# Luckick/EAGCN

Hardware: AMD Instinct MI355X
Metric: molecules/sec fwd+bwd, 2-layer 5-view EAGCN, Tox21 batch (higher is better)
Workload: dtype f32 (bf16x3 split, fp32 accumulate): every fp32 operand leaves its producer as three bf16 planes, six v_mfma_f32_32x32x16_bf16 piece products per 16 k rebuild the fp32 product (csrc/gemm_bx3.hip); aggregation, BatchNorm, head, first layer fp32

## Files before the change

eagcn_amd/_lib.py:

```python
import ctypes as C
import os

_HERE = os.path.dirname(os.path.abspath(__file__))
LIB_PATH = os.path.join(_HERE, 'lib', 'libeagcn_hip.so')

MAX_VIEWS = 8
MAX_SEGS = 8
META_WORDS = 16
META_NLOG = 8
META_T, META_NMAX, META_NTILES, META_BAD_ADJ, META_BAD_REL, META_NEDGE, META_OVERFLOW, META_EDGE_OVERFLOW = range(8)
META_NBLK = 9
STRUCT_CONCATE, STRUCT_WEIGHTED = 0, 1

_fp = C.c_void_p


class Batch(C.Structure):
    _fields_ = [('B', C.c_int32), ('N', C.c_int32), ('K', C.c_int32), ('ldc', C.c_int32),
                ('T', C.c_int32), ('n_max', C.c_int32), ('n_tiles', C.c_int32),
                ('channels', C.c_int32 * MAX_VIEWS),
                ('code', _fp), ('deg_bn', _fp), ('nat', _fp), ('row0', _fp), ('tile0', _fp),
                ('meta', _fp), ('row_mol', _fp), ('row_loc', _fp), ('row_m', _fp), ('row_deg', _fp),
                ('tile_mol', _fp), ('row_info', _fp), ('tile_info', _fp),
                ('rel_vec', _fp * MAX_VIEWS), ('rel_c', C.c_int32 * MAX_VIEWS),
# ... 72 lines not shown

class HeadGrads(C.Structure):
    _fields_ = [(n, _fp) for n in ('d_den1_w', 'd_den2_w', 'd_den3_w', 'd_gbn_w', 'd_gbn_b', 'd_bn1_w', 'd_bn1_b',
                                   'd_bn2_w', 'd_bn2_b')]


class Model(C.Structure):
    _fields_ = [('n_layers', C.c_int32), ('molfp_mode', C.c_int32), ('training', C.c_int32),
                ('head_seed', C.c_uint64), ('head_seed_dev', _fp), ('input_packed', C.c_int32), ('aux_stream', _fp),
                ('layer', LayerParams * 4), ('head', HeadParams), ('stats_hook', _fp), ('stats_user', _fp),
                ('stats_world', C.c_int32), ('fuse_readout', C.c_int32), ('fwd_signal', _fp), ('wait_flag', _fp), ('start_signal', _fp)]


class StepLoss(C.Structure):
    _fields_ = [('kind', C.c_int32), ('labels', _fp), ('class_weight', _fp), ('loss', _fp), ('scale', _fp), ('dout', _fp)]


ALLREDUCE_FN = C.CFUNCTYPE(C.c_int, C.c_void_p, C.c_int, C.c_void_p, C.c_void_p)


SIGNATURES = {
    'eagcn_abi_version': (C.c_int, []),
    'eagcn_struct_size': (C.c_size_t, [C.c_int]),
    'eagcn_last_error': (C.c_char_p, []),
    'eagcn_pad16': (C.c_int, [C.c_int]),
    'eagcn_layer_out_ld': (C.c_int, [C.POINTER(LayerParams)]),
    'eagcn_layer_fp': (C.c_int, [C.POINTER(LayerParams)]),
    'eagcn_layer_packed_bytes': (C.c_size_t, [C.POINTER(Batch), C.POINTER(LayerParams)]),
    'eagcn_layer_fwd_scratch_bytes': (C.c_size_t, [C.POINTER(Batch), C.POINTER(LayerParams)]),
    'eagcn_layer_bwd_scratch_bytes': (C.c_size_t, [C.POINTER(Batch), C.POINTER(LayerParams)]),
    'eagcn_index_build': (C.c_int, [_fp, C.POINTER(_fp), C.POINTER(Batch), _fp, _fp]),
    'eagcn_index_from_bonds': (C.c_int, [_fp, _fp, _fp, _fp, C.c_int64, C.POINTER(Batch), _fp, _fp]),
    'eagcn_index_rows': (C.c_int, [C.POINTER(Batch), _fp]),
    'eagcn_set_gemm_mode': (C.c_int, [C.c_int]),
    'eagcn_stream_wait_counter': (C.c_int, [_fp, C.c_uint32, _fp]),
    'eagcn_stream_signal_flag': (C.c_int, [_fp, _fp]),
    'eagcn_stream_wait_flag': (C.c_int, [_fp, C.c_double, _fp]),
    'eagcn_stream_wait_timeouts': (C.c_int, []),
    'eagcn_stream_wait_reset': (None, []),
    'eagcn_adam_step': (C.c_int, [_fp, _fp, _fp, _fp, C.c_int64, _fp, _fp, _fp, _fp]),
    'eagcn_agg_wants_bond_lists': (C.c_int, [C.c_int, C.c_int]),
    'eagcn_agg_wants_bond_lists_for': (C.c_int, [C.c_int, C.c_int, C.c_int]),
    'eagcn_bx3_used_splits': (C.c_int, [C.c_int, C.c_int, C.c_int, C.c_int]),
    'eagcn_set_bx3_wide': (C.c_int, [C.c_int]),
    'eagcn_bx3_pair_used_splits': (C.c_int, [C.c_int] * 7),
    'eagcn_bx3_plane_elems': (C.c_size_t, [C.c_int, C.c_int]),
    'eagcn_bx3_split': (C.c_int, [_fp, C.c_int, C.c_int, _fp, C.c_size_t, C.c_int, C.c_int, _fp]),
    'eagcn_gemm_bx3': (C.c_int, [C.c_int, C.c_int, C.c_int, C.c_int, _fp, C.c_size_t, C.c_int, C.c_int, _fp, C.c_size_t, C.c_int, C.c_int,
# ... 99 lines not shown
        return _lib
    if not os.path.exists(LIB_PATH):
        raise EagcnHipError(
            'libeagcn_hip.so is not built (%s). Run `python -c "import __graft_entry__ as g; g.build()"` '
            'or `python -m eagcn_amd.build`; eagcn_amd has no CPU fallback.' % LIB_PATH)
    lib = C.CDLL(LIB_PATH)
    lib.eagcn_abi_version.restype = C.c_int
    if lib.eagcn_abi_version() != ABI_VERSION:
        raise EagcnHipError('libeagcn_hip.so speaks ABI version %d, this binding version %d: rebuild it '
                            '(`python -c "import __graft_entry__ as g; g.build()"`)' % (lib.eagcn_abi_version(), ABI_VERSION))
    for name, (res, args) in SIGNATURES.items():
        fn = getattr(lib, name)
        fn.restype = res
        fn.argtypes = args
    for which, cls in ((0, Batch), (1, Layout), (2, LayerParams), (3, LayerBufs), (4, LayerGrads), (5, HeadParams), (6, HeadGrads),
                       (7, Model), (10, StepLoss)):
        if lib.eagcn_struct_size(which) != C.sizeof(cls):
            raise EagcnHipError('ABI mismatch: %s is %d bytes here, %d in libeagcn_hip.so'
                                % (cls.__name__, C.sizeof(cls), lib.eagcn_struct_size(which)))
    _lib = lib
    return lib


def check(rc, what):
    if rc != 0:
        msg = load().eagcn_last_error()
        raise EagcnHipError('%s failed (%d): %s' % (what, rc, msg.decode() if msg else '?'))


def pad16(w):
    return (int(w) + 15) & ~15
# ... 14 lines not shown
```

eagcn_amd/csrc/api.cpp:

```cpp
#include <hip/hip_runtime_api.h>
#include <stdarg.h>
#include <stdint.h>
#include <stdio.h>

#include <vector>

#include "../../include/eagcn_hip.h"

namespace eagcn {
static thread_local char g_err[1024] = "";
void set_error(const char* fmt, ...) {
    va_list ap;
    va_start(ap, fmt);
    vsnprintf(g_err, sizeof(g_err), fmt, ap);
    va_end(ap);
}

hipEvent_t pool_event() {
    static std::vector<hipEvent_t> pool;
    static size_t next = 0;
    constexpr size_t kPool = 256;
    if (pool.empty()) {
        pool.resize(kPool, nullptr);
        for (auto& e : pool)
// ... 59 lines not shown

extern "C" int eagcn_abi_version(void) { return 7; }
extern "C" size_t eagcn_struct_size(int which) {
    switch (which) {
        case 0: return sizeof(eagcn_batch);
        case 1: return sizeof(eagcn_layout);
        case 2: return sizeof(eagcn_layer_params);
        case 3: return sizeof(eagcn_layer_bufs);
        case 4: return sizeof(eagcn_layer_grads);
        case 5: return sizeof(eagcn_head_params);
        case 6: return sizeof(eagcn_head_grads);
        case 7: return sizeof(eagcn_model);
        case 8: return sizeof(eagcn_gat_params);
        case 9: return sizeof(eagcn_pool_att);
        case 10: return sizeof(eagcn_step_loss);
        default: return 0;
    }
}
extern "C" const char* eagcn_last_error(void) { return eagcn::g_err; }
```

eagcn_amd/csrc/head.hip:

```cpp
#include <stdlib.h>

#include <algorithm>

#include "common.h"
#include "kernels.h"

namespace eagcn {

__global__ void wait_counter_kernel(const uint32_t* __restrict__ word, uint32_t value, int* __restrict__ err,
                                    unsigned long long budget_ticks) {
    if (threadIdx.x == 0) {
        const unsigned long long t0 = wall_clock64();
        while ((int32_t)(__hip_atomic_load(word, __ATOMIC_ACQUIRE, __HIP_MEMORY_SCOPE_AGENT) - value) < 0) {
            __builtin_amdgcn_s_sleep(64);
            if (wall_clock64() - t0 > budget_ticks) {
                if (err) __hip_atomic_store(err, 1, __ATOMIC_RELAXED, __HIP_MEMORY_SCOPE_SYSTEM);
                break;
            }
        }
    }
}



// ... 225 lines not shown
    EAGCN_CHECK_ARG(carve_saved(saved, b, m, &sv) <= saved_bytes, "eagcn_model_atom_rep_materialize: saved block too small");
    const int l = m->n_layers - 1;
    LayerSaved& L = sv.L[l];
    eagcn_layer_bufs w;
    memset(&w, 0, sizeof(w));
    w.Y = L.Y; w.bn = L.bn; w.xout = L.xout; w.pad_row = L.pad_row; w.packed = L.packed; w.packed_bytes = L.packed_bytes;
    return layer_apply_impl(b, &m->layer[l], &w, stream);
}

extern "C" int eagcn_model_pack_input(const eagcn_batch* b, const eagcn_model* m, const float* afm, void* saved,
                                      size_t saved_bytes, void* stream) {
    EAGCN_CHECK_ARG(b && m && afm && saved, "eagcn_model_pack_input: null argument");
    ModelSaved sv;
    EAGCN_CHECK_ARG(carve_saved(saved, b, m, &sv) <= saved_bytes, "eagcn_model_pack_input: saved block too small");
    return eagcn_pack_rows(b, afm, layout_width(&m->layer[0].in), &m->layer[0].in, sv.x0, stream);
}

struct HeadPlan {
    HeadFwd f1, f2, f3;
    HeadBwd b3, b2, b1;
    HeadGbn bg;
    double *st_g, *st_1, *st_2, *sb_g, *sb_1, *sb_2;
    bool sync;
};
static HeadPlan head_plan(const eagcn_batch* b, const eagcn_model* m, const ModelSaved& sv, const ModelScratch& sc, float* out,
                          float* graph_rep, const float* dout, const float* dgraph_rep, const eagcn_head_grads* hg) {
    HeadPlan P;
    const eagcn_head_params* h = &m->head;
    const int B = b->B, F = h->f_in, n1 = h->n_den1, n2 = h->n_den2, nc = h->nclass;
    P.st_g = sc.hst; P.st_1 = sc.hst + 2 * F + 2; P.st_2 = sc.hst + 2 * (F + n1) + 4;
// ... 500 lines not shown
```

eagcn_amd/csrc/index.hip:

```cpp
#include <algorithm>

#include <stdlib.h>

#include "common.h"
#include "kernels.h"

namespace eagcn {

struct RelPtrs {
    const float* p[EAGCN_MAX_VIEWS];
    int c[EAGCN_MAX_VIEWS];
};

template <int NIT, int RPW>
__global__ __launch_bounds__(256) void index_scan_kernel(const float* __restrict__ adj, RelPtrs rel,
                                                          int B, int N, int Ncap, int K, int ldc,
                                                          uint8_t* __restrict__ code,
                                                          int32_t* __restrict__ deg_bn,
                                                          int32_t* __restrict__ nat,
                                                          int32_t* __restrict__ ecnt,
                                                          int32_t* __restrict__ meta) {
    const int lane = threadIdx.x & 63;
    const long row_first = ((long)blockIdx.x * 4 + (threadIdx.x >> 6)) * RPW;
    const long nrows = (long)B * N;
// ... 414 lines not shown
        bt.row_loc[r0 + i] = i;
        bt.row_deg[r0 + i] = d;
        bt.row_m[r0 + i] = d > 0 ? 1.0f : 0.0f;
        reinterpret_cast<int4*>(bt.row_info)[r0 + i] = make_int4(b, i, n, r0);
    }
    for (int t = threadIdx.x; t < (n + 15) / 16 && t0 + t < bt.n_tiles; t += blockDim.x) {
        bt.tile_mol[t0 + t] = b;
        reinterpret_cast<int4*>(bt.tile_info)[t0 + t] = make_int4(b, t, n, r0);
    }
    if (threadIdx.x == 0 && bt.mol_info) {
        const int e0 = bt.edge0[b];
        reinterpret_cast<int4*>(bt.mol_info)[b] = make_int4(r0 + n <= bt.T ? n : 0, r0, e0, bt.edge0[b + 1] - e0);
    }
}

__device__ __forceinline__ void index_blocks_body(const eagcn_batch& bt, const int rb, const int lane) {
    const int T = bt.meta[EAGCN_META_T];
    int4* out = reinterpret_cast<int4*>(bt.blk);
    int nb = 0, start = 0, rows = 0, cnt = 0;
    int start_r0 = 0, start_e0 = 0;
    auto close = [&](int end, int end_e0) {
        if (lane == 0) {
            out[2 * nb] = make_int4(start, end - start, start_r0, rows);
            out[2 * nb + 1] = make_int4(start_e0, end_e0 - start_e0, 0, 0);
        }
        ++nb; rows = 0; cnt = 0;
    };
    int last_e0 = 0;
    for (int base = 0; base < bt.B && T > 0; base += 64) {
        const int nv = min(64, bt.B - base);
// ... 182 lines not shown
    return -1;
}

__global__ __launch_bounds__(256) void pack_rows_kernel(eagcn_batch bt, const float* __restrict__ dense,
                                                         int F, ColMap m, int ld, float* __restrict__ packed, int Nin) {
    const uint32_t total = (uint32_t)dev_rows(bt) * (uint32_t)ld;
    for (uint32_t e = blockIdx.x * blockDim.x + threadIdx.x; e < total; e += gridDim.x * blockDim.x) {
        int r = (int)(e / (uint32_t)ld), cp = (int)(e - (uint32_t)r * (uint32_t)ld);
        int ce = packed_to_exact(m, cp);
        float v = 0.0f;
        if (ce >= 0) v = dense[((size_t)bt.row_mol[r] * Nin + bt.row_loc[r]) * F + ce];
        packed[e] = v;
    }
}

__global__ __launch_bounds__(256) void pad_rows_kernel(const float* __restrict__ rows, const int32_t* __restrict__ off,
                                                        int B, int N, int F, float* __restrict__ out) {
    const size_t total = (size_t)B * N * F;
    for (size_t e = (size_t)blockIdx.x * blockDim.x + threadIdx.x; e < total; e += (size_t)gridDim.x * blockDim.x) {
        const int f = (int)(e % F);
        const size_t bi = e / F;
        const int i = (int)(bi % N), b = (int)(bi / N);
        const int o = off[b], n = off[b + 1] - o;
        out[e] = i < n ? rows[(size_t)(o + i) * F + f] : 0.0f;
    }
}

__global__ __launch_bounds__(256) void unpack_rows_kernel(eagcn_batch bt, const float* __restrict__ packed,
                                                           ColMap m, int ld, const float* __restrict__ pad_row,
                                                           float* __restrict__ dense, int F) {
// ... 8 lines not shown
            if (ce < eo + m.w[s]) { cp = po + (ce - eo); break; }
            eo += m.w[s];
            po += m.p[s];
        }
        float v;
        if (i < bt.nat[b]) v = packed[(size_t)(bt.row0[b] + i) * ld + cp];
        else v = pad_row ? pad_row[cp] : 0.0f;
        dense[e] = v;
    }
}

}

using namespace eagcn;

extern "C" int eagcn_index_build(const float* adj, const float* const* rel, eagcn_batch* b,
                                 int32_t* host_meta, void* stream) {
    hipStream_t s = (hipStream_t)stream;
    EAGCN_CHECK_ARG(adj && rel && b && host_meta, "eagcn_index_build: null argument");
    EAGCN_CHECK_ARG(b->B > 0 && b->N > 0, "eagcn_index_build: B and N must be positive");
    EAGCN_CHECK_ARG(b->K >= 1 && b->K <= EAGCN_MAX_VIEWS, "eagcn_index_build: K=%d out of range", b->K);
    EAGCN_CHECK_ARG(b->ldc >= b->N && (b->ldc % 16) == 0, "eagcn_index_build: ldc must be a multiple of 16 >= N");
    EAGCN_CHECK_ARG(b->code && b->deg_bn && b->nat && b->row0 && b->tile0 && b->meta,
                    "eagcn_index_build: index buffers not allocated");
    RelPtrs rp;
    for (int k = 0; k < EAGCN_MAX_VIEWS; ++k) {
        rp.p[k] = k < b->K ? rel[k] : nullptr;
        rp.c[k] = k < b->K ? b->channels[k] : 0;
        if (k < b->K) {
            EAGCN_CHECK_ARG(rel[k] != nullptr, "eagcn_index_build: relation tensor %d is null", k);
            EAGCN_CHECK_ARG(rp.c[k] >= 1 && rp.c[k] <= EAGCN_MAX_CHANNELS,
                            "eagcn_index_build: view %d has %d channels (1..%d supported)", k, rp.c[k],
// ... 26 lines not shown
#undef EAGCN_SCAN4
#undef EAGCN_SCAN4_AL
        EAGCN_LAUNCH_CHECK();
    } else
    {
#define EAGCN_SCAN(NIT) index_scan_kernel<NIT, RPW><<<sgrid, 256, 0, s>>>(adj, rp, b->B, Nin, b->N, b->K, b->ldc, b->code, b->deg_bn, b->nat, b->ecnt, b->meta)
        switch (nit) {
            case 1: EAGCN_SCAN(1); break;
            case 2: EAGCN_SCAN(2); break;
            case 3: EAGCN_SCAN(3); break;
            default: EAGCN_SCAN(4); break;
        }
#undef EAGCN_SCAN
        EAGCN_LAUNCH_CHECK();
    }
    index_offsets_kernel<<<1, 1024, 0, s>>>(b->nat, b->B, b->deg_bn, b->B * b->N, b->row0, b->tile0, b->meta, b->T, b->ecnt, b->edge0, b->E, b->n_logical > 0 ? b->n_logical : 0);
    EAGCN_LAUNCH_CHECK();
    EAGCN_HIP(hipMemcpyAsync(host_meta, b->meta, EAGCN_META_WORDS * sizeof(int32_t), hipMemcpyDeviceToHost, s));
    return EAGCN_OK;
}

extern "C" int eagcn_index_from_bonds(const int32_t* bond_mol, const int32_t* bond_i, const int32_t* bond_j,
                                      const uint8_t* bond_code, int64_t E, eagcn_batch* b, int32_t* host_meta,
                                      void* stream) {
    hipStream_t s = (hipStream_t)stream;
    EAGCN_CHECK_ARG(b && host_meta, "eagcn_index_from_bonds: null argument");
    EAGCN_CHECK_ARG(E == 0 || (bond_mol && bond_i && bond_j && bond_code), "eagcn_index_from_bonds: null bond arrays");
    EAGCN_CHECK_ARG(b->B > 0 && b->N > 0 && b->K >= 1 && b->K <= EAGCN_MAX_VIEWS, "eagcn_index_from_bonds: bad batch shape");
    EAGCN_CHECK_ARG(b->ldc >= b->N && (b->ldc % 16) == 0, "eagcn_index_from_bonds: ldc must be a multiple of 16 >= N");
    EAGCN_CHECK_ARG(b->code && b->deg_bn && b->nat && b->row0 && b->tile0 && b->meta,
                    "eagcn_index_from_bonds: index buffers not allocated");
    RelPtrs rp;
    for (int k = 0; k < EAGCN_MAX_VIEWS; ++k) { rp.p[k] = nullptr; rp.c[k] = k < b->K ? b->channels[k] : 0; }
    ProfScope ps(PROF_INDEX, s);
    EAGCN_CHECK_ARG(b->ecnt && b->edge0, "eagcn_index_from_bonds: bond-list buffers not allocated");
    EAGCN_CHECK_ARG((long)b->B * b->N < (1L << 31), "eagcn_index_from_bonds: B * N = %ld rows", (long)b->B * b->N);
    {
        const int rcz = index_clear(b->meta, b->nat, b->ecnt, b->B, b->deg_bn, (long)b->B * b->N, s);
        if (rcz) return rcz;
    }
    EAGCN_HIP(hipMemsetAsync(b->code, 0, (size_t)b->K * b->B * b->N * b->ldc, s));
    if (E > 0) {
        const int grid = (int)std::min<long>((E + 255) / 256, 4096);
        index_bonds_kernel<<<grid, 256, 0, s>>>(bond_mol, bond_i, bond_j, bond_code, (long)E, b->B, b->N,
                                                b->n_logical > 0 ? std::min(b->n_logical, b->N) : b->N, b->K, b->ldc, rp,
                                                b->code, b->deg_bn, b->nat, b->ecnt, b->meta);
        EAGCN_LAUNCH_CHECK();
    }
    index_offsets_kernel<<<1, 1024, 0, s>>>(b->nat, b->B, b->deg_bn, b->B * b->N, b->row0, b->tile0, b->meta, b->T, b->ecnt, b->edge0, b->E, b->n_logical > 0 ? b->n_logical : 0);
    EAGCN_LAUNCH_CHECK();
    EAGCN_HIP(hipMemcpyAsync(host_meta, b->meta, EAGCN_META_WORDS * sizeof(int32_t), hipMemcpyDeviceToHost, s));
    return EAGCN_OK;
}

extern "C" int eagcn_index_rows(const eagcn_batch* b, void* stream) {
    hipStream_t s = (hipStream_t)stream;
    EAGCN_CHECK_ARG(b, "eagcn_index_rows: null batch");
    if (b->T == 0) return EAGCN_OK;
    EAGCN_CHECK_ARG(b->row_mol && b->row_loc && b->row_m && b->row_deg && b->tile_mol && b->row_info && b->tile_info,
                    "eagcn_index_rows: per-row buffers not allocated");
    EAGCN_CHECK_ARG(b->N <= 1024, "eagcn_index_rows: N=%d exceeds the supported 1024 atoms", b->N);
    EAGCN_CHECK_ARG(b->edge0 && b->mol_info && b->row_ptr && b->col_ptr && (b->E == 0 || (b->nbr && b->tnbr && b->ecode && b->tcode)),
                    "eagcn_index_rows: bond-list buffers not allocated");
    ProfScope ps(PROF_INDEX, s);
    index_rows_kernel<<<b->B, 256, 0, s>>>(*b);
    EAGCN_LAUNCH_CHECK();
    if (!b->build_lists) return EAGCN_OK;
    const int rb = b->blk ? lagg_block_rows(b) : 0;
    const int W = (b->N + 31) / 32;
    const size_t dyn = (size_t)2 * b->N * W * sizeof(uint32_t);
    static const size_t lds_cap = [] {
        int dev = 0, v = 0;
        if (hipGetDevice(&dev) != hipSuccess || hipDeviceGetAttribute(&v, hipDeviceAttributeMaxSharedMemoryPerBlock, dev) != hipSuccess) v = 64 * 1024;
        size_t cap = (size_t)v > 12 * 1024 ? (size_t)v - 12 * 1024 : 0;
        if (cap > 52 * 1024 &&
            hipFuncSetAttribute((const void*)index_csr_kernel<true>, hipFuncAttributeMaxDynamicSharedMemorySize, (int)cap) != hipSuccess) {
            (void)hipGetLastError();
            cap = 52 * 1024;
        }
        return cap;
    }();
    if (b->N <= 512 && dyn <= lds_cap) index_csr_kernel<true><<<b->B + (rb > 0 ? 1 : 0), 256, dyn, s>>>(*b, W, rb);
    else index_csr_kernel<false><<<b->B + (rb > 0 ? 1 : 0), 256, 0, s>>>(*b, W, rb);
    EAGCN_LAUNCH_CHECK();
    return EAGCN_OK;
}

extern "C" int eagcn_pack_rows(const eagcn_batch* b, const float* dense, int F, const eagcn_layout* lay,
                               float* packed, void* stream) {
    hipStream_t s = (hipStream_t)stream;
    EAGCN_CHECK_ARG(b && dense && lay && packed, "eagcn_pack_rows: null argument");
    EAGCN_CHECK_ARG(layout_width(lay) == F, "eagcn_pack_rows: layout width %d != F %d", layout_width(lay), F);
    if (b->T == 0) return EAGCN_OK;
    int ld = layout_ld(lay);
    size_t total = (size_t)b->T * ld;
    int grid = (int)std::min<size_t>((total + 255) / 256, 4096);
    ProfScope ps(PROF_PACK, s);
    pack_rows_kernel<<<grid, 256, 0, s>>>(*b, dense, F, make_colmap(lay), ld, packed, b->n_logical > 0 ? b->n_logical : b->N);
    EAGCN_LAUNCH_CHECK();
    return EAGCN_OK;
}
// ... 26 lines not shown
```

eagcn_amd/csrc/kernels.h:

```cpp
#pragma once
#include "bx3.h"
#include "common.h"

namespace eagcn {

struct AggArgs {
    eagcn_batch bt;
    ViewCols vc;
    const float* src; int lds;
    float* dst; int ldd;
    const float* sig;
    const float* rsig;
    float* rscale;
    double* stats;
    int nchunk;
    int cpw = 1;
    int xcd = 0;
    bool w_rowm = false;
    BxOut planes = {nullptr, 0, 0, 0};
    const float* bn_tab = nullptr; const float* bn_cc = nullptr; int bn_fp = 0;
    const float* w_aw = nullptr;
    int w_drop = 0; uint32_t w_thr = 0; float w_inv_keep = 1.0f; uint64_t w_seed = 0; const uint64_t* w_seed_dev = nullptr;
};
int agg_grid_x(const eagcn_batch* b);
bool agg_ksplit(const eagcn_batch* b);
int launch_agg(AggArgs a, bool trans, hipStream_t s);
constexpr int LAGG_RB = 256;
constexpr int LAGG_MAXM = 16;
struct EdgeArgs;
int lagg_parts();
bool lagg_wfuse();
bool lagg_use(const eagcn_batch* b, int dir, bool absorbs_bn, const ViewCols* vc = nullptr);
bool lagg_wanted(int B, int N, int structure);
int lagg_block_rows(const eagcn_batch* b);
int lagg_slabs(const eagcn_batch* b);
int launch_lagg_fwd(AggArgs a, hipStream_t s);
int launch_lagg_bwd(AggArgs a, const EdgeArgs& e, hipStream_t s, bool edge = true);
int launch_lagg_bwd_input(const AggArgs& a, const EdgeArgs& e, dim3 grid, hipStream_t s);

struct EdgeArgs {
    eagcn_batch bt;
    ViewCols vc;
    const float* dY; const float* Y; const float* P; int ld;
    const float* sig; const float* rsig; const float* rscale;
    double* datt;
    int atomic;
    int xcd = 0;
};
constexpr int EDGE_SLAB = 264;
constexpr int EDGE_COPIES = 8;
inline size_t edge_acc_bytes() { return align256((size_t)EDGE_COPIES * EAGCN_MAX_VIEWS * EDGE_SLAB * sizeof(double)); }
// ... 192 lines not shown
```

eagcn_amd/graph.py:

```python
import ctypes as C
import os

import torch

from . import _lib as L
from . import ops
from .ops import _index_stream, _ptr, _stream

_RING = 4
_SIDE_AFTER_FWD = os.environ.get('EAGCN_SIDE_AFTER_FWD', '1') == '1'
_SIDE_PLACED = os.environ.get('EAGCN_SIDE_PLACED', '0')
_SIDE_PLACED_MAX_ROWS = int(os.environ.get('EAGCN_SIDE_PLACED_MAX_ROWS', '40000'))
_REQUIRE_IN_GRAPH = os.environ.get('EAGCN_REQUIRE_IN_GRAPH_ALLREDUCE', '0') == '1'
_COMM_IN_GRAPH = os.environ.get('EAGCN_COMM_IN_GRAPH', '1') != '0'
_CAPTURE_DRAIN_S = float(os.environ.get('EAGCN_CAPTURE_DRAIN_S', '0.35'))


_READY_FLAG = os.environ.get('EAGCN_READY_FLAG', '1') != '0'
_flag_tested = {}


def _ready_flag_ok(device):
    if not _READY_FLAG:
        return False
    key = device.index if device.index is not None else torch.cuda.current_device()
    if key not in _flag_tested:
        lib = L.load()
        flag = torch.zeros(1, dtype=torch.int32, device=device)
        torch.cuda.synchronize(device)
        main, side = torch.cuda.current_stream(device), _index_stream(device)
        L.check(lib.eagcn_stream_wait_flag(C.c_void_p(flag.data_ptr()), 0.05, C.c_void_p(main.cuda_stream)), 'eagcn_stream_wait_flag')
        L.check(lib.eagcn_stream_signal_flag(C.c_void_p(flag.data_ptr()), C.c_void_p(side.cuda_stream)), 'eagcn_stream_signal_flag')
        torch.cuda.synchronize(device)
# ... 91 lines not shown
        self.generation = 0
        self.size_static = [torch.ones(B, dtype=torch.int64, device=device) for _ in range(2)]
        self.aux = None
        self.dp_group = None
        if os.environ.get('EAGCN_AUX_STREAM', '0') == '1':
            self.aux = torch.cuda.Stream(device=self.device)
        self.fwd_sig = torch.zeros(1, dtype=torch.int32, device=device)
        self.side_placed = _SIDE_PLACED == '1' or (_SIDE_PLACED == 'auto' and B * N <= _SIDE_PLACED_MAX_ROWS)
        self.ready = torch.zeros(2, dtype=torch.int32, device=device)
        self.use_flag = _ready_flag_ok(device)
        self.start_word = torch.zeros(1, dtype=torch.int32, device=device)
        self.starts_issued = 0
        self.markers = [None, None]
        self.fwd_issued = 0
        self.cms = [self._cmodel(i) for i in range(2)]
        m = self.cms[0]
        self.saved_bytes = lib.eagcn_model_saved_bytes(self.index.ref(), C.byref(m))
        self.scratch_bytes = lib.eagcn_model_scratch_bytes(self.index.ref(), C.byref(m))
        self.saved = [torch.empty(self.saved_bytes, dtype=torch.uint8, device=device) for _ in range(2)]
        self.scratch = torch.empty(self.scratch_bytes, dtype=torch.uint8, device=device)
        if plan.stats is not None:
            from .parallel import register_stats_buffer
            register_stats_buffer(self.scratch)
        f32 = dict(dtype=torch.float32, device=device)
        self.out = torch.zeros((B, m.head.nclass), **f32)
        self.graph_rep = torch.zeros((B, m.head.n_den2), **f32)
        self.dout = torch.zeros((B, m.head.nclass), **f32)
        self.dgr = torch.zeros((B, m.head.n_den2), **f32)
        self.dgr_is_zero = True
        self._weight_src = None
# ... 158 lines not shown
        lib = L.load()
        self._check_old_batches()
        self.cur = cur = self.step % 2
        idx = self.index = self.slots[cur]
        main = torch.cuda.current_stream(self.device)
        slot = self.step % _RING
        if self.meta_event[slot] is not None:
            self._check_old_batches(force=True, only=slot)
        if self.use_flag:
            slot_free = ('count', self.starts_issued) if self.starts_issued >= 2 else None
        else:
            ev = torch.cuda.Event()
            ev.record(main)
            slot_free = self.markers[1]
            self.markers = [self.markers[1], ('event', ev)]
        if overlap:
            side = _index_stream(self.device)
            if slot_free is not None and slot_free[0] == 'event':
                side.wait_event(slot_free[1])
            elif slot_free is not None:
                L.check(lib.eagcn_stream_wait_counter(C.c_void_p(self.start_word.data_ptr()), slot_free[1] & 0xFFFFFFFF,
                                                      C.c_void_p(side.cuda_stream)), 'eagcn_stream_wait_counter')
            if self.fwd_done is not None and _SIDE_AFTER_FWD:
                side.wait_event(self.fwd_done)
            elif self.side_placed and self.fwd_issued > 0:
                L.check(lib.eagcn_stream_wait_counter(C.c_void_p(self.fwd_sig.data_ptr()), self.fwd_issued & 0xFFFFFFFF,
                                                      C.c_void_p(side.cuda_stream)), 'eagcn_stream_wait_counter')
            for t in (afm, adj, size, labels) + tuple(rels or ()) + tuple(bonds or ()):
                if isinstance(t, torch.Tensor) and t.is_cuda:
                    t.record_stream(side)
        else:
            side = main
        istream = C.c_void_p(side.cuda_stream)
        idx.c.n_logical = int(self.n_in) if self.n_in != idx.N else 0
        if bonds is None:
            rel_ptrs = (C.c_void_p * idx.K)(*[r.data_ptr() for r in rels])
            L.check(lib.eagcn_index_build(_ptr(adj), rel_ptrs, idx.ref(), C.c_void_p(self.meta_host[slot].data_ptr()),
                                          istream), 'eagcn_index_build')
        else:
            bm, bi, bj, bc = bonds
            L.check(lib.eagcn_index_from_bonds(_ptr(bm), _ptr(bi), _ptr(bj), _ptr(bc), bm.numel(), idx.ref(),
                                               C.c_void_p(self.meta_host[slot].data_ptr()), istream),
                    'eagcn_index_from_bonds')
        L.check(lib.eagcn_index_rows(idx.ref(), istream), 'eagcn_index_rows')
        L.check(lib.eagcn_model_pack_input(idx.ref(), C.byref(self.cms[cur]), _ptr(afm), _ptr(self.saved[cur]),
                                           self.saved_bytes, istream), 'eagcn_model_pack_input')
        sh = self.seeds_host[slot]
        sn = sh.numpy()
        for l in range(4):
# ... 33 lines not shown
            if bad:
                if overlap:
                    main.wait_stream(side)
                raise L.EagcnHipError(bad)
        if self.use_flag:
            L.check(lib.eagcn_stream_signal_flag(C.c_void_p(self.ready.data_ptr() + 4 * cur), istream), 'eagcn_stream_signal_flag')
        elif overlap:
            done = torch.cuda.Event()
            done.record(side)
            main.wait_event(done)
        self.step += 1
        self.generation += 1
        if self.training:
            self.plan.nbt_pending += 1
        return main

    def _set_row_hint(self):
        if self.t_hint is None:
            slot = (self.step - 1) % _RING
            ev = self.meta_event[slot]
            if ev is not None:
                ev.synchronize()
            t = int(self.meta_host[slot][L.META_T])
            self.t_hint = max(1, min(t, self.index.T)) if t > 0 else 0
        for sl in self.slots:
            sl.c.t_hint = self.t_hint

    def _reset_ready(self):
        if self.use_flag:
            torch.cuda.synchronize(self.device)
# ... 296 lines not shown
```

include/eagcn_hip.h:

```cpp
#ifndef EAGCN_HIP_H
#define EAGCN_HIP_H

#include <stddef.h>
#include <stdint.h>

#ifdef __cplusplus
extern "C" {
#endif

#define EAGCN_MAX_VIEWS 8
#define EAGCN_MAX_SEGS 8
#define EAGCN_MAX_CHANNELS 255
#define EAGCN_STRUCT_CONCATE 0
#define EAGCN_STRUCT_WEIGHTED 1

#define EAGCN_OK 0
#define EAGCN_ERR_ARG (-1)
#define EAGCN_ERR_HIP (-2)
#define EAGCN_ERR_SCRATCH (-3)

#define EAGCN_META_T 0
#define EAGCN_META_NMAX 1
#define EAGCN_META_NTILES 2
#define EAGCN_META_BAD_ADJ 3
// ... 217 lines not shown

int eagcn_stream_signal_flag(uint32_t* flag, void* stream);
int eagcn_stream_wait_flag(uint32_t* flag, double budget_seconds, void* stream);
int eagcn_stream_wait_timeouts(void);
void eagcn_stream_wait_reset(void);

int eagcn_stream_wait_counter(const uint32_t* counter, uint32_t value, void* stream);

size_t eagcn_model_saved_bytes(const eagcn_batch* b, const eagcn_model* m);
size_t eagcn_model_scratch_bytes(const eagcn_batch* b, const eagcn_model* m);
int eagcn_model_atom_rep(const eagcn_batch* b, const eagcn_model* m, size_t* xout_offset,
                         size_t* pad_row_offset, int* ld);
int eagcn_model_atom_rep_materialize(const eagcn_batch* b, const eagcn_model* m, void* saved, size_t saved_bytes, void* stream);
int eagcn_model_pack_input(const eagcn_batch* b, const eagcn_model* m, const float* afm, void* saved,
                           size_t saved_bytes, void* stream);
int eagcn_model_forward(const eagcn_batch* b, const eagcn_model* m, const float* afm, const int64_t* size,
                        void* saved, size_t saved_bytes, void* scratch, size_t scratch_bytes, float* out,
                        float* graph_rep, void* stream);
int eagcn_model_backward(const eagcn_batch* b, const eagcn_model* m, const int64_t* size, void* saved,
                         size_t saved_bytes, void* scratch, size_t scratch_bytes, const float* dout,
                         const float* dgraph_rep, const eagcn_layer_grads* lg, const eagcn_head_grads* hg,
                         void* stream);

int eagcn_model_backward_range(const eagcn_batch* b, const eagcn_model* m, const int64_t* size, void* saved,
                               size_t saved_bytes, void* scratch, size_t scratch_bytes, const float* dout,
                               const float* dgraph_rep, const eagcn_layer_grads* lg, const eagcn_head_grads* hg,
                               int with_head, int layer_hi, int layer_lo, void* stream);

size_t eagcn_model_input_scratch_bytes(const eagcn_batch* b, const eagcn_model* m);
int eagcn_model_backward_input(const eagcn_batch* b, const eagcn_model* m, const int64_t* size, void* saved,
// ... 92 lines not shown
```

Baseline: 691,000.

## Fuse per-batch index tail, input packing and side copies into one native prepare call

Adds eagcn_batch_prepare, a single native entry point that issues the stream waits, the index build, a new fused offsets+rows kernel, and one kernel that packs the input rows while also writing the dropout seeds and performing the small staging copies. The Python step uses it by default in place of many separate ctypes calls, torch copies and kernel launches. The goal is to cut per-step host overhead and launch count on the side stream. The cost is that the fused offsets kernel has every block re-reduce the prefix over all earlier molecules, which is O(B^2) work in total. It also adds a new ABI struct and a second code path to keep consistent with the legacy one.

```diff
diff --git a/eagcn_amd/_lib.py b/eagcn_amd/_lib.py
--- a/eagcn_amd/_lib.py
+++ b/eagcn_amd/_lib.py
@@ -110,6 +110,19 @@
 
 class StepLoss(C.Structure):
     _fields_ = [('kind', C.c_int32), ('labels', _fp), ('class_weight', _fp), ('loss', _fp), ('scale', _fp), ('dout', _fp)]
+
+
+PREPARE_MAX_COPIES = 12
+
+
+class PrepareArgs(C.Structure):
+    _fields_ = [('batch', C.POINTER(Batch)), ('model', C.POINTER(Model)), ('adj', _fp), ('rel', C.POINTER(_fp)),
+                ('bond_mol', _fp), ('bond_i', _fp), ('bond_j', _fp), ('bond_code', _fp), ('n_bonds', C.c_int64),
+                ('afm', _fp), ('saved', _fp), ('saved_bytes', C.c_size_t), ('free_word', _fp), ('fwd_word', _fp),
+                ('free_value', C.c_uint32), ('fwd_value', C.c_uint32), ('seeds_dev', _fp), ('seeds', C.c_int64 * 8),
+                ('n_copies', C.c_int32), ('reserved_', C.c_int32), ('copy_dst', _fp * PREPARE_MAX_COPIES),
+                ('copy_src', _fp * PREPARE_MAX_COPIES), ('copy_words', C.c_int64 * PREPARE_MAX_COPIES), ('ready', _fp),
+                ('host_meta', _fp)]
 
 
 ALLREDUCE_FN = C.CFUNCTYPE(C.c_int, C.c_void_p, C.c_int, C.c_void_p, C.c_void_p)
@@ -128,6 +141,7 @@
     'eagcn_index_build': (C.c_int, [_fp, C.POINTER(_fp), C.POINTER(Batch), _fp, _fp]),
     'eagcn_index_from_bonds': (C.c_int, [_fp, _fp, _fp, _fp, C.c_int64, C.POINTER(Batch), _fp, _fp]),
     'eagcn_index_rows': (C.c_int, [C.POINTER(Batch), _fp]),
+    'eagcn_batch_prepare': (C.c_int, [C.POINTER(PrepareArgs), _fp]),
     'eagcn_set_gemm_mode': (C.c_int, [C.c_int]),
     'eagcn_stream_wait_counter': (C.c_int, [_fp, C.c_uint32, _fp]),
     'eagcn_stream_signal_flag': (C.c_int, [_fp, _fp]),
@@ -257,7 +271,7 @@
         fn.restype = res
         fn.argtypes = args
     for which, cls in ((0, Batch), (1, Layout), (2, LayerParams), (3, LayerBufs), (4, LayerGrads), (5, HeadParams), (6, HeadGrads),
-                       (7, Model), (10, StepLoss)):
+                       (7, Model), (10, StepLoss), (11, PrepareArgs)):
         if lib.eagcn_struct_size(which) != C.sizeof(cls):
             raise EagcnHipError('ABI mismatch: %s is %d bytes here, %d in libeagcn_hip.so'
                                 % (cls.__name__, C.sizeof(cls), lib.eagcn_struct_size(which)))
diff --git a/eagcn_amd/csrc/api.cpp b/eagcn_amd/csrc/api.cpp
--- a/eagcn_amd/csrc/api.cpp
+++ b/eagcn_amd/csrc/api.cpp
@@ -97,6 +97,7 @@
         case 8: return sizeof(eagcn_gat_params);
         case 9: return sizeof(eagcn_pool_att);
         case 10: return sizeof(eagcn_step_loss);
+        case 11: return sizeof(eagcn_prepare_args);
         default: return 0;
     }
 }
diff --git a/eagcn_amd/csrc/head.hip b/eagcn_amd/csrc/head.hip
--- a/eagcn_amd/csrc/head.hip
+++ b/eagcn_amd/csrc/head.hip
@@ -263,6 +263,13 @@
     ModelSaved sv;
     EAGCN_CHECK_ARG(carve_saved(saved, b, m, &sv) <= saved_bytes, "eagcn_model_pack_input: saved block too small");
     return eagcn_pack_rows(b, afm, layout_width(&m->layer[0].in), &m->layer[0].in, sv.x0, stream);
+}
+
+namespace eagcn {
+float* model_input_slot(const eagcn_batch* b, const eagcn_model* m, void* saved, size_t saved_bytes) {
+    ModelSaved sv;
+    return carve_saved(saved, b, m, &sv) <= saved_bytes ? sv.x0 : nullptr;
+}
 }
 
 struct HeadPlan {
diff --git a/eagcn_amd/csrc/index.hip b/eagcn_amd/csrc/index.hip
--- a/eagcn_amd/csrc/index.hip
+++ b/eagcn_amd/csrc/index.hip
@@ -452,6 +452,64 @@
     }
 }
 
+__global__ __launch_bounds__(256) void index_rows_off_kernel(eagcn_batch bt, int n_logical) {
+    __shared__ int s_part[4][4];
+    const int b = blockIdx.x, tid = threadIdx.x;
+    const int lim = b == 0 ? bt.B : b;
+    int sr = 0, st = 0, se = 0, mx = 0;
+    for (int i = tid; i < lim; i += 256) {
+        const int v = bt.nat[i];
+        sr += v;
+        st += (v + 15) >> 4;
+        se += bt.ecnt[i];
+        mx = max(mx, v);
+    }
+    sr = wave_sum(sr); st = wave_sum(st); se = wave_sum(se);
+#pragma unroll
+    for (int o = 32; o > 0; o >>= 1) mx = max(mx, __shfl_xor(mx, o));
+    if ((tid & 63) == 0) { s_part[tid >> 6][0] = sr; s_part[tid >> 6][1] = st; s_part[tid >> 6][2] = se; s_part[tid >> 6][3] = mx; }
+    __syncthreads();
+    sr = s_part[0][0] + s_part[1][0] + s_part[2][0] + s_part[3][0];
+    st = s_part[0][1] + s_part[1][1] + s_part[2][1] + s_part[3][1];
+    se = s_part[0][2] + s_part[1][2] + s_part[2][2] + s_part[3][2];
+    mx = max(max(s_part[0][3], s_part[1][3]), max(s_part[2][3], s_part[3][3]));
+    const int n = bt.nat[b], ne = bt.ecnt[b];
+    const int r0 = b == 0 ? 0 : sr, t0 = b == 0 ? 0 : st, e0 = b == 0 ? 0 : se;
+    if (tid == 0) {
+        bt.row0[b] = r0;
+        bt.tile0[b] = t0;
+        bt.edge0[b] = e0;
+        if (b == 0) {
+            bt.row0[bt.B] = sr;
+            bt.tile0[bt.B] = st;
+            bt.edge0[bt.B] = se;
+            const bool over_r = bt.T > 0 && sr > bt.T;
+            const bool over_e = se > bt.E;
+            const bool over = over_r || over_e;
+            bt.meta[EAGCN_META_NEDGE] = se;
+            bt.meta[EAGCN_META_T] = over ? 0 : sr;
+            bt.meta[EAGCN_META_NTILES] = over ? 0 : st;
+            bt.meta[EAGCN_META_OVERFLOW] = over_r ? sr : 0;
+            bt.meta[EAGCN_META_EDGE_OVERFLOW] = over_e ? se : 0;
+            bt.meta[EAGCN_META_NMAX] = mx;
+            bt.meta[EAGCN_META_NLOG] = n_logical;
+        }
+    }
+    for (int i = tid; i < n && r0 + i < bt.T; i += 256) {
+        int d = bt.deg_bn[(size_t)b * bt.N + i];
+        bt.row_mol[r0 + i] = b;
+        bt.row_loc[r0 + i] = i;
+        bt.row_deg[r0 + i] = d;
+        bt.row_m[r0 + i] = d > 0 ? 1.0f : 0.0f;
+        reinterpret_cast<int4*>(bt.row_info)[r0 + i] = make_int4(b, i, n, r0);
+    }
+    for (int t = tid; t < (n + 15) / 16 && t0 + t < bt.n_tiles; t += 256) {
+        bt.tile_mol[t0 + t] = b;
+        reinterpret_cast<int4*>(bt.tile_info)[t0 + t] = make_int4(b, t, n, r0);
+    }
+    if (tid == 0 && bt.mol_info) reinterpret_cast<int4*>(bt.mol_info)[b] = make_int4(r0 + n <= bt.T ? n : 0, r0, e0, ne);
+}
+
 __device__ __forceinline__ void index_blocks_body(const eagcn_batch& bt, const int rb, const int lane) {
     const int T = bt.meta[EAGCN_META_T];
     int4* out = reinterpret_cast<int4*>(bt.blk);
@@ -664,6 +722,38 @@
     }
 }
 
+struct PrepRiders {
+    int64_t seeds[8];
+    int64_t* seeds_dev;
+    int n_copies;
+    uint32_t* dst[EAGCN_PREPARE_MAX_COPIES];
+    const uint32_t* src[EAGCN_PREPARE_MAX_COPIES];
+    long words[EAGCN_PREPARE_MAX_COPIES];
+};
+__global__ __launch_bounds__(256) void pack_prepare_kernel(eagcn_batch bt, const float* __restrict__ dense, int F, ColMap m, int ld,
+                                                            float* __restrict__ packed, int Nin, int pack_blocks, PrepRiders x) {
+    const int blk = blockIdx.x;
+    if (blk < pack_blocks) {
+        const uint32_t total = (uint32_t)dev_rows(bt) * (uint32_t)ld;
+        for (uint32_t e = blk * 256 + threadIdx.x; e < total; e += (uint32_t)pack_blocks * 256) {
+            int r = (int)(e / (uint32_t)ld), cp = (int)(e - (uint32_t)r * (uint32_t)ld);
+            int ce = packed_to_exact(m, cp);
+            float v = 0.0f;
+            if (ce >= 0) v = dense[((size_t)bt.row_mol[r] * Nin + bt.row_loc[r]) * F + ce];
+            packed[e] = v;
+        }
+    } else if (blk == pack_blocks) {
+        if (threadIdx.x == 0 && x.seeds_dev) {
+#pragma unroll
+            for (int i = 0; i < 8; ++i) x.seeds_dev[i] = x.seeds[i];
+        }
+    } else {
+        const long first = (long)(blk - pack_blocks - 1) * 256 + threadIdx.x, stride = (long)(gridDim.x - pack_blocks - 1) * 256;
+        for (int c = 0; c < x.n_copies; ++c)
+            for (long i = first; i < x.words[c]; i += stride) x.dst[c][i] = x.src[c][i];
+    }
+}
+
 __global__ __launch_bounds__(256) void pad_rows_kernel(const float* __restrict__ rows, const int32_t* __restrict__ off,
                                                         int B, int N, int F, float* __restrict__ out) {
     const size_t total = (size_t)B * N * F;
@@ -702,8 +792,7 @@
 
 using namespace eagcn;
 
-extern "C" int eagcn_index_build(const float* adj, const float* const* rel, eagcn_batch* b,
-                                 int32_t* host_meta, void* stream) {
+static int index_build_impl(const float* adj, const float* const* rel, eagcn_batch* b, int32_t* host_meta, void* stream, bool tail) {
     hipStream_t s = (hipStream_t)stream;
     EAGCN_CHECK_ARG(adj && rel && b && host_meta, "eagcn_index_build: null argument");
     EAGCN_CHECK_ARG(b->B > 0 && b->N > 0, "eagcn_index_build: B and N must be positive");
@@ -760,15 +849,20 @@
 #undef EAGCN_SCAN
         EAGCN_LAUNCH_CHECK();
     }
+    if (!tail) return EAGCN_OK;
     index_offsets_kernel<<<1, 1024, 0, s>>>(b->nat, b->B, b->deg_bn, b->B * b->N, b->row0, b->tile0, b->meta, b->T, b->ecnt, b->edge0, b->E, b->n_logical > 0 ? b->n_logical : 0);
     EAGCN_LAUNCH_CHECK();
     EAGCN_HIP(hipMemcpyAsync(host_meta, b->meta, EAGCN_META_WORDS * sizeof(int32_t), hipMemcpyDeviceToHost, s));
     return EAGCN_OK;
 }
-
-extern "C" int eagcn_index_from_bonds(const int32_t* bond_mol, const int32_t* bond_i, const int32_t* bond_j,
-                                      const uint8_t* bond_code, int64_t E, eagcn_batch* b, int32_t* host_meta,
-                                      void* stream) {
+extern "C" int eagcn_index_build(const float* adj, const float* const* rel, eagcn_batch* b,
+                                 int32_t* host_meta, void* stream) {
+    return index_build_impl(adj, rel, b, host_meta, stream, true);
+}
+
+static int index_from_bonds_impl(const int32_t* bond_mol, const int32_t* bond_i, const int32_t* bond_j,
+                                 const uint8_t* bond_code, int64_t E, eagcn_batch* b, int32_t* host_meta,
+                                 void* stream, bool tail) {
     hipStream_t s = (hipStream_t)stream;
     EAGCN_CHECK_ARG(b && host_meta, "eagcn_index_from_bonds: null argument");
     EAGCN_CHECK_ARG(E == 0 || (bond_mol && bond_i && bond_j && bond_code), "eagcn_index_from_bonds: null bond arrays");
@@ -793,13 +887,19 @@
                                                 b->code, b->deg_bn, b->nat, b->ecnt, b->meta);
         EAGCN_LAUNCH_CHECK();
     }
+    if (!tail) return EAGCN_OK;
     index_offsets_kernel<<<1, 1024, 0, s>>>(b->nat, b->B, b->deg_bn, b->B * b->N, b->row0, b->tile0, b->meta, b->T, b->ecnt, b->edge0, b->E, b->n_logical > 0 ? b->n_logical : 0);
     EAGCN_LAUNCH_CHECK();
     EAGCN_HIP(hipMemcpyAsync(host_meta, b->meta, EAGCN_META_WORDS * sizeof(int32_t), hipMemcpyDeviceToHost, s));
     return EAGCN_OK;
 }
-
-extern "C" int eagcn_index_rows(const eagcn_batch* b, void* stream) {
+extern "C" int eagcn_index_from_bonds(const int32_t* bond_mol, const int32_t* bond_i, const int32_t* bond_j,
+                                      const uint8_t* bond_code, int64_t E, eagcn_batch* b, int32_t* host_meta,
+                                      void* stream) {
+    return index_from_bonds_impl(bond_mol, bond_i, bond_j, bond_code, E, b, host_meta, stream, true);
+}
+
+static int index_rows_impl(const eagcn_batch* b, void* stream, bool offsets) {
     hipStream_t s = (hipStream_t)stream;
     EAGCN_CHECK_ARG(b, "eagcn_index_rows: null batch");
     if (b->T == 0) return EAGCN_OK;
@@ -809,7 +909,8 @@
     EAGCN_CHECK_ARG(b->edge0 && b->mol_info && b->row_ptr && b->col_ptr && (b->E == 0 || (b->nbr && b->tnbr && b->ecode && b->tcode)),
                     "eagcn_index_rows: bond-list buffers not allocated");
     ProfScope ps(PROF_INDEX, s);
-    index_rows_kernel<<<b->B, 256, 0, s>>>(*b);
+    if (offsets) index_rows_off_kernel<<<b->B, 256, 0, s>>>(*b, b->n_logical > 0 ? b->n_logical : 0);
+    else index_rows_kernel<<<b->B, 256, 0, s>>>(*b);
     EAGCN_LAUNCH_CHECK();
     if (!b->build_lists) return EAGCN_OK;
     const int rb = b->blk ? lagg_block_rows(b) : 0;
@@ -831,6 +932,56 @@
     EAGCN_LAUNCH_CHECK();
     return EAGCN_OK;
 }
+extern "C" int eagcn_index_rows(const eagcn_batch* b, void* stream) { return index_rows_impl(b, stream, false); }
+
+extern "C" int eagcn_batch_prepare(const eagcn_prepare_args* a, void* stream) {
+    hipStream_t s = (hipStream_t)stream;
+    EAGCN_CHECK_ARG(a && a->batch && a->model && a->afm && a->saved && a->host_meta, "eagcn_batch_prepare: null argument");
+    eagcn_batch* b = a->batch;
+    EAGCN_CHECK_ARG(b->T > 0, "eagcn_batch_prepare: the batch has no row capacity");
+    EAGCN_CHECK_ARG(a->n_copies >= 0 && a->n_copies <= EAGCN_PREPARE_MAX_COPIES, "eagcn_batch_prepare: %d copies (at most %d)",
+                    a->n_copies, EAGCN_PREPARE_MAX_COPIES);
+    PrepRiders x;
+    long copy_words = 0;
+    for (int c = 0; c < EAGCN_PREPARE_MAX_COPIES; ++c) {
+        const bool live = c < a->n_copies;
+        if (live)
+            EAGCN_CHECK_ARG(a->copy_dst[c] && a->copy_src[c] && a->copy_words[c] >= 0 &&
+                            ((reinterpret_cast<uintptr_t>(a->copy_dst[c]) | reinterpret_cast<uintptr_t>(a->copy_src[c])) & 3) == 0,
+                            "eagcn_batch_prepare: copy %d is null, negative or not 4-byte aligned", c);
+        x.dst[c] = live ? static_cast<uint32_t*>(a->copy_dst[c]) : nullptr;
+        x.src[c] = live ? static_cast<const uint32_t*>(a->copy_src[c]) : nullptr;
+        x.words[c] = live ? (long)a->copy_words[c] : 0;
+        copy_words += x.words[c];
+    }
+    x.n_copies = a->n_copies;
+    x.seeds_dev = a->seeds_dev;
+    for (int i = 0; i < 8; ++i) x.seeds[i] = a->seeds[i];
+    const eagcn_layout* lay = &a->model->layer[0].in;
+    float* x0 = model_input_slot(b, a->model, a->saved, a->saved_bytes);
+    EAGCN_CHECK_ARG(x0 != nullptr, "eagcn_batch_prepare: saved block too small");
+    if (a->free_word) { const int rc = eagcn_stream_wait_counter(a->free_word, a->free_value, stream); if (rc) return rc; }
+    if (a->fwd_word) { const int rc = eagcn_stream_wait_counter(a->fwd_word, a->fwd_value, stream); if (rc) return rc; }
+    {
+        const int rc = a->adj ? index_build_impl(a->adj, a->rel, b, a->host_meta, stream, false)
+                              : index_from_bonds_impl(a->bond_mol, a->bond_i, a->bond_j, a->bond_code, a->n_bonds, b, a->host_meta, stream, false);
+        if (rc) return rc;
+    }
+    { const int rc = index_rows_impl(b, stream, true); if (rc) return rc; }
+    {
+        const int F = layout_width(lay), ld = layout_ld(lay);
+        const size_t total = (size_t)b->T * ld;
+        const int pack_blocks = (int)std::min<size_t>((total + 255) / 256, 4096);
+        const int copy_blocks = copy_words > 0 ? (int)std::min<long>((copy_words + 1023) / 1024, 64) : 0;
+        ProfScope ps(PROF_PACK, s);
+        pack_prepare_kernel<<<pack_blocks + 1 + copy_blocks, 256, 0, s>>>(*b, a->afm, F, make_colmap(lay), ld, x0,
+                                                                          b->n_logical > 0 ? b->n_logical : b->N, pack_blocks, x);
+        EAGCN_LAUNCH_CHECK();
+    }
+    if (a->ready) { const int rc = eagcn_stream_signal_flag(a->ready, stream); if (rc) return rc; }
+    EAGCN_HIP(hipMemcpyAsync(a->host_meta, b->meta, EAGCN_META_WORDS * sizeof(int32_t), hipMemcpyDeviceToHost, s));
+    return EAGCN_OK;
+}
 
 extern "C" int eagcn_pack_rows(const eagcn_batch* b, const float* dense, int F, const eagcn_layout* lay,
                                float* packed, void* stream) {
diff --git a/eagcn_amd/csrc/kernels.h b/eagcn_amd/csrc/kernels.h
--- a/eagcn_amd/csrc/kernels.h
+++ b/eagcn_amd/csrc/kernels.h
@@ -35,6 +35,7 @@
 int lagg_block_rows(const eagcn_batch* b);
 int lagg_slabs(const eagcn_batch* b);
 int launch_lagg_fwd(AggArgs a, hipStream_t s);
+float* model_input_slot(const eagcn_batch* b, const eagcn_model* m, void* saved, size_t saved_bytes);
 int launch_lagg_bwd(AggArgs a, const EdgeArgs& e, hipStream_t s, bool edge = true);
 int launch_lagg_bwd_input(const AggArgs& a, const EdgeArgs& e, dim3 grid, hipStream_t s);
 
diff --git a/eagcn_amd/graph.py b/eagcn_amd/graph.py
--- a/eagcn_amd/graph.py
+++ b/eagcn_amd/graph.py
@@ -17,6 +17,7 @@
 
 
 _READY_FLAG = os.environ.get('EAGCN_READY_FLAG', '1') != '0'
+_PREPARE = os.environ.get('EAGCN_PREPARE', 'native')
 _flag_tested = {}
 
 
@@ -138,6 +139,7 @@
         self.markers = [None, None]
         self.fwd_issued = 0
         self.cms = [self._cmodel(i) for i in range(2)]
+        self._prep_args = [None, None]
         m = self.cms[0]
         self.saved_bytes = lib.eagcn_model_saved_bytes(self.index.ref(), C.byref(m))
         self.scratch_bytes = lib.eagcn_model_scratch_bytes(self.index.ref(), C.byref(m))
@@ -326,15 +328,21 @@
             ev.record(main)
             slot_free = self.markers[1]
             self.markers = [self.markers[1], ('event', ev)]
+        native = self.use_flag and _PREPARE != 'legacy' and self.validate != 'sync' and not isinstance(dp_scale, str)
+        waits = [None, None]
         if overlap:
             side = _index_stream(self.device)
             if slot_free is not None and slot_free[0] == 'event':
                 side.wait_event(slot_free[1])
+            elif slot_free is not None and native:
+                waits[0] = (self.start_word, slot_free[1] & 0xFFFFFFFF)
             elif slot_free is not None:
                 L.check(lib.eagcn_stream_wait_counter(C.c_void_p(self.start_word.data_ptr()), slot_free[1] & 0xFFFFFFFF,
                                                       C.c_void_p(side.cuda_stream)), 'eagcn_stream_wait_counter')
             if self.fwd_done is not None and _SIDE_AFTER_FWD:
                 side.wait_event(self.fwd_done)
+            elif self.side_placed and self.fwd_issued > 0 and native:
+                waits[1] = (self.fwd_sig, self.fwd_issued & 0xFFFFFFFF)
             elif self.side_placed and self.fwd_issued > 0:
                 L.check(lib.eagcn_stream_wait_counter(C.c_void_p(self.fwd_sig.data_ptr()), self.fwd_issued & 0xFFFFFFFF,
                                                       C.c_void_p(side.cuda_stream)), 'eagcn_stream_wait_counter')
@@ -345,6 +353,13 @@
             side = main
         istream = C.c_void_p(side.cuda_stream)
         idx.c.n_logical = int(self.n_in) if self.n_in != idx.N else 0
+        if native:
+            self._prepare_native(adj, rels, afm, size, seed, bonds, labels, dp_scale, side, waits, slot)
+            self.step += 1
+            self.generation += 1
+            if self.training:
+                self.plan.nbt_pending += 1
+            return main
         if bonds is None:
             rel_ptrs = (C.c_void_p * idx.K)(*[r.data_ptr() for r in rels])
             L.check(lib.eagcn_index_build(_ptr(adj), rel_ptrs, idx.ref(), C.c_void_p(self.meta_host[slot].data_ptr()),
@@ -408,6 +423,64 @@
         if self.training:
             self.plan.nbt_pending += 1
         return main
+
+    def _prepare_native(self, adj, rels, afm, size, seed, bonds, labels, dp_scale, side, waits, slot):
+        lib = L.load()
+        cur, idx = self.cur, self.index
+        a = self._prep_args[cur]
+        if a is None:
+            a = self._prep_args[cur] = L.PrepareArgs()
+            a.batch, a.model = C.pointer(idx.c), C.pointer(self.cms[cur])
+            a.saved, a.saved_bytes = self.saved[cur].data_ptr(), self.saved_bytes
+            a.seeds_dev = self.seeds_dev[cur].data_ptr()
+            a.ready = self.ready.data_ptr() + 4 * cur
+            a._rel = (C.c_void_p * idx.K)()
+        pairs = []
+        if self.plan.molfp:
+            pairs.append((self.size_static[cur], size))
+        if labels is not None:
+            pairs.append((self.labels_static[cur], labels.reshape(self.labels_static[cur].shape)))
+        if dp_scale is not None:
+            pairs.append((self.scale_static[cur], dp_scale))
+        if idx.relvec is not None:
+            pairs += [(t[:v.shape[0]], v) for t, v in zip(idx.relvec, self.rel_vectors)]
+        n, by_torch = 0, []
+        for dst, src in pairs:
+            if (isinstance(src, torch.Tensor) and src.device == dst.device and src.dtype == dst.dtype and src.is_contiguous()
+                    and src.shape == dst.shape and n < L.PREPARE_MAX_COPIES):
+                a.copy_dst[n], a.copy_src[n], a.copy_words[n] = dst.data_ptr(), src.data_ptr(), dst.numel() * dst.element_size() // 4
+                n += 1
+            else:
+                by_torch.append((dst, src))
+        a.n_copies = n
+        istream = C.c_void_p(side.cuda_stream)
+        if by_torch:
+            for w in waits:
+                if w is not None:
+                    L.check(lib.eagcn_stream_wait_counter(C.c_void_p(w[0].data_ptr()), w[1], istream), 'eagcn_stream_wait_counter')
+            waits = [None, None]
+            with torch.cuda.stream(side):
+                for dst, src in by_torch:
+                    dst.copy_(src, non_blocking=True)
+        a.free_word, a.free_value = (waits[0][0].data_ptr(), waits[0][1]) if waits[0] else (None, 0)
+        a.fwd_word, a.fwd_value = (waits[1][0].data_ptr(), waits[1][1]) if waits[1] else (None, 0)
+        if bonds is None:
+            for k, r in enumerate(rels):
+                a._rel[k] = r.data_ptr()
+            a.adj, a.rel = adj.data_ptr(), C.cast(a._rel, C.POINTER(C.c_void_p))
+        else:
+            bm, bi, bj, bc = bonds
+            a.adj, a.rel = None, None
+            a.bond_mol, a.bond_i, a.bond_j, a.bond_code, a.n_bonds = bm.data_ptr(), bi.data_ptr(), bj.data_ptr(), bc.data_ptr(), bm.numel()
+        a.afm = afm.data_ptr()
+        for l in range(4):
+            a.seeds[l] = (seed + 7919 * (l + 1)) & (2 ** 63 - 1)
+        a.seeds[4] = (seed + 0x51ED27) & (2 ** 63 - 1)
+        a.host_meta = self.meta_host[slot].data_ptr()
+        L.check(lib.eagcn_batch_prepare(C.byref(a), istream), 'eagcn_batch_prepare')
+        ev = torch.cuda.Event()
+        ev.record(side)
+        self.meta_event[slot] = ev
 
     def _set_row_hint(self):
         if self.t_hint is None:
diff --git a/include/eagcn_hip.h b/include/eagcn_hip.h
--- a/include/eagcn_hip.h
+++ b/include/eagcn_hip.h
@@ -255,6 +255,37 @@
 int eagcn_model_atom_rep_materialize(const eagcn_batch* b, const eagcn_model* m, void* saved, size_t saved_bytes, void* stream);
 int eagcn_model_pack_input(const eagcn_batch* b, const eagcn_model* m, const float* afm, void* saved,
                            size_t saved_bytes, void* stream);
+
+#define EAGCN_PREPARE_MAX_COPIES 12
+typedef struct eagcn_prepare_args {
+    eagcn_batch* batch;
+    const eagcn_model* model;
+    const float* adj;
+    const float* const* rel;
+    const int32_t* bond_mol;
+    const int32_t* bond_i;
+    const int32_t* bond_j;
+    const uint8_t* bond_code;
+    int64_t n_bonds;
+    const float* afm;
+    void* saved;
+    size_t saved_bytes;
+    const uint32_t* free_word;
+    const uint32_t* fwd_word;
+    uint32_t free_value;
+    uint32_t fwd_value;
+    int64_t* seeds_dev;
+    int64_t seeds[8];
+    int32_t n_copies;
+    int32_t reserved_;
+    void* copy_dst[EAGCN_PREPARE_MAX_COPIES];
+    const void* copy_src[EAGCN_PREPARE_MAX_COPIES];
+    int64_t copy_words[EAGCN_PREPARE_MAX_COPIES];
+    uint32_t* ready;
+    int32_t* host_meta;
+} eagcn_prepare_args;
+int eagcn_batch_prepare(const eagcn_prepare_args* a, void* stream);
+
 int eagcn_model_forward(const eagcn_batch* b, const eagcn_model* m, const float* afm, const int64_t* size,
                         void* saved, size_t saved_bytes, void* scratch, size_t scratch_bytes, float* out,
                         float* graph_rep, void* stream);
```

After: 685,800. About the same (-0.8%).
